# lawmurray/BayesLogit

Measured on NVIDIA B200. Metric: pg_draws_per_sec, higher is better.
Workload: dtype f64

## Files before the change

bayeslogit_b200/api.py:

```python
import ctypes as C

import numpy as np

from . import _lib

NA = float("nan")


def set_seed(seed):
    _lib.lib().bl_set_seed(int(seed) & 0xFFFFFFFFFFFFFFFF)


def set_device(device):
    _lib.check(_lib.lib().bl_set_device(int(device)))


def _recycle(a, num, dtype):
    a = np.asarray(a, dtype=dtype).ravel()
    if a.size != num:
        a = np.resize(a, num)
    return np.ascontiguousarray(a)


def _ptr(a):
# ... 100 lines not shown
    z = np.ascontiguousarray(z, dtype=np.float64)
    shape = np.ascontiguousarray(shape, dtype=dt)
    num = z.size
    x = np.zeros(num)
    t = _lib.Tape()
    keep = []
    for k in "ueng":
        a = tape.get(k)
        if a is None:
            setattr(t, "t" + k, None)
            setattr(t, "l" + k, 0)
        else:
            a = np.ascontiguousarray(a, dtype=np.float64)
            assert a.ndim == 2 and a.shape[0] == num
            keep.append(a)
            setattr(t, "t" + k, a.ctypes.data)
            setattr(t, "l" + k, a.shape[1])
    tr = np.zeros((num, _lib.TRACE_W), dtype=np.int32) if trace else None
    args = [_ptr(x), _ptr(shape), _ptr(z), num]
    it = None
    if method == "gamma":
        args.append(int(trunc))
    if method == "sp":
        it = np.zeros(num, dtype=np.int32)
        args.append(_ptr(it))
    st = getattr(_lib.lib(), fn)(*args, C.byref(t), _ptr(tr) if trace else None)
    _lib.check(st)
    out = [x]
    if trace:
        out.append(tr)
    if it is not None:
        out.append(it)
    return tuple(out) if len(out) > 1 else x


def pg_moments(b, z):
    b = np.ascontiguousarray(b, dtype=np.float64)
    z = np.ascontiguousarray(z, dtype=np.float64)
    m1, m2 = np.zeros(b.size), np.zeros(b.size)
    _lib.check(_lib.lib().bl_probe_pg_moments(_ptr(m1), _ptr(m2), _ptr(b), _ptr(z), b.size))
    return m1, m2


def v_eval(y):
    y = np.ascontiguousarray(y, dtype=np.float64)
    v = np.zeros(y.size)
    _lib.check(_lib.lib().bl_probe_v_eval(_ptr(v), _ptr(y), y.size))
    return v


SPECFUN = {"p_norm": 0, "log_p_norm": 1, "p_gamma_rate": 2, "p_igauss": 3, "lgamma": 4, "tgamma": 5,
           "dev_right_mass": 6, "dev_coef": 7, "upper_gamma_cf": 8, "p_igauss_direct": 9, "sp_log_cos_rt": 10,
           "sp_v_table": 11, "sp_pl": 12, "sp_pl_estimate": 13,
           "alt_pr": 14, "alt_pr_estimate": 15}


def specfun(which, a, b=None, c=None):
    a = np.ascontiguousarray(a, dtype=np.float64)
    b = a if b is None else np.ascontiguousarray(np.broadcast_to(b, a.shape), dtype=np.float64)
    c = a if c is None else np.ascontiguousarray(np.broadcast_to(c, a.shape), dtype=np.float64)
    out = np.zeros(a.size)
    _lib.check(_lib.lib().bl_probe_specfun(_ptr(out), SPECFUN[which], _ptr(a), _ptr(b), _ptr(c), a.size))
    return out


def philox4x32_10(ctr, key):
    ctr = np.ascontiguousarray(ctr, dtype=np.uint32)
    key = np.ascontiguousarray(key, dtype=np.uint32)
    out = np.zeros(4, dtype=np.uint32)
    _lib.check(_lib.lib().bl_probe_philox(_ptr(out), _ptr(ctr), _ptr(key)))
    return out
```

bayeslogit_b200/csrc/pg_alt.cuh:

```cuda
#pragma once

namespace bl {

template <class Src>
__device__ __forceinline__ double alt_rtinvchi2(Src &s, double h, double trunc)
{
    double h2 = h * h;
    double R = trunc / h2;
    double E1 = s.expon();
    double E2 = s.expon();
    while ((E1 * E1) > (2 * E2 / R)) {
        E1 = s.expon();
        E2 = s.expon();
    }
    double X = 1 + E1 * R;
    X = R / (X * X);
    return h2 * X;
}

__device__ __forceinline__ double alt_pigauss(double x, double z, double lambda)
{
    double sq = sqrt(lambda / x);
    double b = sq * (x * z - 1);
    double a = sq * (x * z + 1) * -1.0;
    return p_norm(b) + ool::exp_(2 * lambda * z) * p_norm(a);
}

enum AltField {
    kAltH = 0,
    kAltTrunc,
    kAltPr,
    kAltCoef,
    kAltLgh,
    kAltLd0, kAltLd1,
    kAltLtB, kAltLtC0, kAltLtLM,
    kAltPrBand,
    kAltSetupDoubles
};
constexpr int kAltStateDoubles = 2 * kAltSetupDoubles;

struct AltState {
    double f[kAltStateDoubles];
    __device__ __forceinline__ double get(int k) const { return f[k]; }
};

struct AltStateRef {
    const double *o;
    size_t stride;
    __device__ __forceinline__ double get(int k) const { return o[(size_t)k * stride]; }
};

__device__ __forceinline__ void alt_plan(double h, int &nfull, int &nrem, double &hrem)
{
    double n = floor((h - 1.0) / 4.0);
    double remain = h - 4.0 * n;
    nfull = (int)n;
    if (remain > 4.0) {
        nrem = 2;
        hrem = 0.5 * remain;
    } else {
        nrem = 1;
        hrem = remain;
    }
}

static __device__ __noinline__ double alt_pr_fp64(double h, double z, double trunc)
{
    const double kLog2 = 0.693147180559945309417232;
    double wl, wr;
    if (z != 0)
        wl = ool::exp_(h * (kLog2 - z)) * alt_pigauss(trunc, z / h, h * h);
    else
        wl = ool::exp_(h * kLog2) * (1.0 - p_gamma_rate(1 / trunc, 0.5, 0.5 * h * h));
    double lambda_z = kPi * kPi * 0.125 + 0.5 * z * z;
    wr = ool::exp_(h * ool::log_((0.5 * kPi) / lambda_z)) * (1.0 - p_gamma_rate(trunc, h, lambda_z));
    return wr / (wr + wl);
}

constexpr double kAltPrBandWidth = 2e-5;

__device__ __forceinline__ float alt_pr_estimate(double h, double z, double trunc)
{
    const float hf = (float)h, zf = (float)z, tf = (float)trunc;
    if (!(zf < 12.0f)) return -1.0f;
    const float s = hf * rsqrtf(tf);
    const float tz = tf * zf / hf;
    const float b = s * (tz - 1.0f), na = s * (tz + 1.0f);
    const float phib = 0.5f * erfcf(-b * 0.70710678f);
    const float wl = exp2f(hf) * (__expf(-hf * zf) * phib
                                  + 0.5f * erfcxf(na * 0.70710678f) * __expf(hf * zf - 0.5f * na * na));
    const float lam = 1.2337005501361697f + 0.5f * zf * zf;
    const float x = tf * lam;
    const float lpre = hf * __logf(x) - x;
    float Q;
    if (x < hf + 1.0f) {
        float term = 1.0f, sum = 1.0f, ap = hf;
        for (int k = 0; k < 60; ++k) {
            ap += 1.0f;
            term *= x / ap;
            sum += term;
            if (term < 1e-8f * sum) break;
        }
        Q = 1.0f - sum * __expf(lpre - lgammaf(hf + 1.0f));
    } else {
        float cf = upper_gamma_cf_f32(hf, x);
        if (!(cf > 0.0f)) return -1.0f;
        Q = cf * __expf(lpre - lgammaf(hf));
    }
    if (!(Q > 0.0f)) return -1.0f;
    const float wr = __expf(hf * __logf(1.5707963267948966f / lam)) * Q;
    const float pr = wr / (wr + wl);
    return pr >= 0.0f && pr <= 1.0f ? pr : -1.0f;
}

template <bool kEstimatePr>
static __device__ __noinline__ void alt_setup(double h, double z, double *out)
{
    const double kLog2 = 0.693147180559945309417232;
    int idx = (int)floor((h - 1.0) * 100.0);
    double trunc = PG_TRUNC_SCHEDULE[idx];
    double rate_z = 0.125 * kPi * kPi + 0.5 * z * z;
    float est = kEstimatePr ? alt_pr_estimate(h, z, trunc) : -1.0f;
    out[kAltH] = h;
    out[kAltTrunc] = trunc;
    out[kAltPr] = est >= 0.0f ? (double)est : alt_pr_fp64(h, z, trunc);
    out[kAltPrBand] = est >= 0.0f ? kAltPrBandWidth : 0.0;
    out[kAltCoef] = ool::exp_(h * kLog2 - 0.5 * 1.8378770664093454835606594728112 );
    out[kAltLgh] = ool::lgamma_(h);
    out[kAltLd0] = ool::log_(h);
    out[kAltLd1] = ool::log_(2.0 + h);
    double b = rate_z * trunc;
    double d1 = b - h;
    double d3 = h - 1.0;
    double c0 = 0.5 * (d1 + sqrt(d1 * d1 + 4.0 * b)) / b;
    out[kAltLtB] = b;
    out[kAltLtC0] = c0;
    out[kAltLtLM] = d3 * ool::log_(d3 / (1.0 - c0)) - d3;
}

template <class St>
__device__ __forceinline__ bool alt_pick_right(double u, const St &st, int o, double z)
{
    const double pr = st.get(o + kAltPr), band = st.get(o + kAltPrBand);
    if (u < pr - band) return true;
    if (u > pr + band || band == 0.0) return false;
    return u < alt_pr_fp64(st.get(o + kAltH), z, st.get(o + kAltTrunc));
}

struct AltLane {
    double X, alpha, sum;
    int trial;
    int phase;
    int nfull;
    int nrem;
    __device__ __forceinline__ void start(int nf, int nr)
    {
        X = 0.0; alpha = 0.0; sum = 0.0; trial = 0; phase = 0; nfull = nf; nrem = nr;
    }
};

__device__ __forceinline__ double alt_coef(double n, double lx3, double ldn, double x, double h,
                                           double coef_h, double &g)
{
    double d_n = 2.0 * n + h;
    if (n != 0)
        g *= (n + h - 1) / n;
    else
        g = 1.0;
    double coef = coef_h * g;
    double log_kernel = -0.5 * (lx3 + d_n * d_n / x) + ldn;
    return coef * ool::exp_(log_kernel);
}

template <class Src, class St>
__device__ __forceinline__ bool alt_pick(Src &src, AltLane &L, double z, const St &st)
{
    const int o = L.nfull > 0 ? 0 : kAltSetupDoubles;
    if (L.trial >= 10000) {
        L.sum += -1.0;
        L.trial = 0;
        if (L.nfull > 0)
            L.nfull--;
        else
            L.nrem--;
        return L.nfull == 0 && L.nrem == 0;
    }
    L.trial++;
    if (alt_pick_right(src.unif(), st, o, z)) {
        L.phase = 1;
    } else {
// ... 80 lines not shown
    const double trunc = st.get(o + kAltTrunc);
    bool chunk_done = false;
    double chunk_val = 0.0;
    if (L.phase == 1) {
        double rate_z = 0.125 * kPi * kPi + 0.5 * z * z;
        if (h == 1.0) {
            L.X = src.expon() / rate_z + trunc;
            L.phase = 4;
        } else {
            double b = st.get(o + kAltLtB), c0 = st.get(o + kAltLtC0);
            double x = b + src.expon() / c0;
            double u = src.unif();
            double l_rho = (h - 1.0) * ool::log_(x) - x * (1.0 - c0);
            if (ool::log_(u) <= l_rho - st.get(o + kAltLtLM)) {
                L.X = trunc * (x / b);
                L.phase = 4;
            }
        }
    } else if (L.phase == 2) {
        if (src.unif() > L.alpha) {
            L.X = alt_rtinvchi2(src, h, trunc);
            L.alpha = ool::exp_(-0.5 * z * z * L.X);
        } else {
            L.phase = 4;
        }
    } else if (L.phase == 3) {
        double X = igauss(src, h / z, h * h);
        if (!(X > trunc)) {
            L.X = X;
            L.phase = 4;
        }
    }
    if (L.phase == 4) {
        const double X = L.X;
        const bool accept = alt_series_test(X, src.unif(), h, trunc, st, o);
        L.phase = 0;
        if (accept) {
            chunk_done = true;
            chunk_val = 0.25 * X;
        }
    }
    if (chunk_done) {
        L.sum += chunk_val;
        L.trial = 0;
        if (L.nfull > 0)
            L.nfull--;
        else
            L.nrem--;
        if (L.nfull == 0 && L.nrem == 0) return true;
    }
    return false;
}

template <class Src>
__device__ double alt_draw(Src &s, double h, double z)
{
    if (h < 1) return 0;
    if (h != h) return h;
    int nfull, nrem;
    double hrem;
    alt_plan(h, nfull, nrem, hrem);
    double zh = fabs(z) * 0.5;
    AltState st;
    if (nfull > 0) alt_setup<false>(4.0, zh, st.f);
    alt_setup<false>(hrem, zh, st.f + kAltSetupDoubles);
    AltLane L;
    L.start(nfull, nrem);
    while (!alt_trip(s, L, zh, st)) {}
    return L.sum;
}

}
```

bayeslogit_b200/csrc/pg_hybrid.cu:

```cuda
#include <algorithm>
#include <cstdlib>
#include <vector>

#include "engine.h"
#include "pg_devroye_fast.cuh"
#include "pg_stream.cuh"

namespace bl {

namespace {

constexpr int kBinThreads = 256;
constexpr int kMetaCounts = 0;
constexpr int kMetaOffsets = 8;
constexpr int kMetaCursor = 16;

__global__ void __launch_bounds__(kBinThreads)
k_hyb_count(const double *__restrict__ h, int n, int *__restrict__ meta)
{
    __shared__ int cnt[8];
    if (threadIdx.x < 8) cnt[threadIdx.x] = 0;
    __syncthreads();
    int local[6] = {0, 0, 0, 0, 0, 0};
    for (int i = blockIdx.x * blockDim.x + threadIdx.x; i < n; i += gridDim.x * blockDim.x)
// ... 125 lines not shown
struct RgSlots {
    double f[F][kRgThreads];
    double d[D][kRgThreads];
    uint4 buf[kRgThreads];
    uint32_t blk[kRgThreads];
    int pos[kRgThreads];
    int i[I][kRgThreads];
    int obs[kRgThreads];
    int phase[kRgThreads];
    int perm[kRgThreads];
    int wcnt[kRgThreads / 32][3];
};

struct SpRegroup {
    static constexpr int F = kSpStateDoubles, D = 3, I = 1, kClasses = 2, kRegime = kRegSP;
    using Slots = RgSlots<F, D, I>;
    __device__ static void begin(Slots &S, int t, double shape, double zraw, PhiloxSource &src)
    {
        S.d[0][t] = shape;
        S.d[1][t] = 0.5 * fabs(zraw);
        S.d[2][t] = 2.0;
        S.i[0][t] = 1;
        SpStateRef st{&S.f[0][t], (size_t)kRgThreads};
        S.phase[t] = sp_pick_left(src.unif(), st, shape) ? 1 : 2;
    }
    __device__ static bool advance(Slots &S, int sl, PhiloxSource &src, double &omega)
    {
        SpLane L;
        L.X = S.d[2][sl];
        L.iter = S.i[0][sl];
        L.phase = S.phase[sl];
        const double n = S.d[0][sl];
        SpStateRef st{&S.f[0][sl], (size_t)kRgThreads};
        bool done = sp_trip_staged(src, L, n, S.d[1][sl], st);
        if (!done && L.phase == 0) {
            if (L.iter >= 200) {
                done = true;
            } else {
                L.iter++;
                L.phase = sp_pick_left(src.unif(), st, n) ? 1 : 2;
            }
        }
        if (done) {
            omega = n * 0.25 * L.X;
        } else {
            S.d[2][sl] = L.X;
            S.i[0][sl] = L.iter;
            S.phase[sl] = L.phase;
        }
        return done;
    }
};

struct AltRegroup {
    static constexpr int F = kAltStateDoubles, D = 4, I = 3, kClasses = 3, kRegime = kRegAlt;
    using Slots = RgSlots<F, D, I>;
    __device__ static void load(const Slots &S, int sl, AltLane &L)
    {
        L.X = S.d[1][sl]; L.alpha = S.d[2][sl]; L.sum = S.d[3][sl];
        L.trial = S.i[0][sl]; L.nfull = S.i[1][sl]; L.nrem = S.i[2][sl];
        L.phase = S.phase[sl];
    }
    __device__ static void store(Slots &S, int sl, const AltLane &L)
    {
        S.d[1][sl] = L.X; S.d[2][sl] = L.alpha; S.d[3][sl] = L.sum;
        S.i[0][sl] = L.trial; S.i[1][sl] = L.nfull; S.i[2][sl] = L.nrem;
        S.phase[sl] = L.phase;
    }
    __device__ static void begin(Slots &S, int t, double shape, double zraw, PhiloxSource &src)
    {
        int nfull, nrem;
        double hrem;
        alt_plan(shape, nfull, nrem, hrem);
        AltLane L;
        L.start(nfull, nrem);
        const double zh = 0.5 * fabs(zraw);
        S.d[0][t] = zh;
        AltStateRef st{&S.f[0][t], (size_t)kRgThreads};
        alt_pick(src, L, zh, st);
        store(S, t, L);
    }
    __device__ static bool advance(Slots &S, int sl, PhiloxSource &src, double &omega)
    {
        AltLane L;
        load(S, sl, L);
        const double zh = S.d[0][sl];
        AltStateRef st{&S.f[0][sl], (size_t)kRgThreads};
        bool done = alt_trip<false>(src, L, zh, st);
        while (!done && L.phase == 0) done = alt_pick(src, L, zh, st);
        if (done)
            omega = L.sum;
        else
            store(S, sl, L);
        return done;
    }
};

template <class R, bool kChains = false>
__global__ void __launch_bounds__(kRgThreads)
k_loop_regroup(double *__restrict__ x, const double *__restrict__ h, const double *__restrict__ z,
               const int *__restrict__ idx, const int *__restrict__ meta, const double *__restrict__ state,
               int c0, int cap, StreamId id)
{
    using Slots = typename R::Slots;
    extern __shared__ __align__(16) unsigned char rg_raw[];
    Slots &S = *reinterpret_cast<Slots *>(rg_raw);
    const int count = min(meta[kMetaCounts + R::kRegime] - c0, cap);
    if (count <= 0) return;
    const int *list = idx + meta[kMetaOffsets + R::kRegime] + c0;
    const unsigned full = 0xffffffffu;
    const int t = threadIdx.x, lane = t & 31, warp = t >> 5;
    const unsigned lt_mask = (1u << lane) - 1u;
    constexpr int kWarps = kRgThreads / 32;
    const int gwarp = blockIdx.x * kWarps + warp;
    const int stride = gridDim.x * kWarps * kLaneChunk;
    int cur = gwarp * kLaneChunk, cend = cur + kLaneChunk;

    S.phase[t] = -1;
    __syncthreads();
    for (;;) {
        const bool empty = S.phase[t] < 0;
        const unsigned want = __ballot_sync(full, empty);
        if (want && cur < count) {
            int rank = __popc(want & lt_mask);
            int cand = cur + rank;
            if (cand >= cend) cand += stride - kLaneChunk;
            if (empty && cand < count) {
                const int obs = list[cand];
#pragma unroll
                for (int k = 0; k < R::F; ++k) S.f[k][t] = __ldg(state + (size_t)k * cap + cand);
                S.obs[t] = obs;
                PhiloxSource src;
                if (kChains) open_batch_stream(src, id, obs);
                else src.open(id.seed, id.obs0 + (uint64_t)obs, id.call_id);
                R::begin(S, t, h[obs], z[obs], src);
                S.buf[t] = src.buf;
                S.blk[t] = src.blk;
                S.pos[t] = src.pos;
            }
            cur += __popc(want);
            if (cur >= cend) {
// ... 15 lines not shown
            tot1 += a;
            tot2 += b;
            tot3 += c;
        }
        if (tot1 + tot2 + tot3 == 0) {
            if (!__syncthreads_or(cur < count)) break;
            continue;
        }
        if (ph == 1) S.perm[b1 + __popc(m1 & lt_mask)] = t;
        else if (ph == 3) S.perm[tot1 + b3 + __popc(m3 & lt_mask)] = t;
        else if (ph == 2) S.perm[kRgThreads - 1 - (b2 + __popc(m2 & lt_mask))] = t;
        __syncthreads();
        if (t < tot1 + tot3 || t >= kRgThreads - tot2) {
            const int sl = S.perm[t];
            PhiloxSource src;
            if (kChains) open_batch_stream(src, id, S.obs[sl]);
            else src.open(id.seed, id.obs0 + (uint64_t)S.obs[sl], id.call_id);
            src.buf = S.buf[sl];
            src.blk = S.blk[sl];
            src.pos = S.pos[sl];
            double omega;
            if (R::advance(S, sl, src, omega)) {
                x[S.obs[sl]] = omega;
                S.phase[sl] = -1;
            } else {
                S.buf[sl] = src.buf;
                S.blk[sl] = src.blk;
                S.pos[sl] = src.pos;
            }
        }
        __syncthreads();
    }
}

template <class R, bool kChains>
int regroup_grid()
{
    using Slots = typename R::Slots;
    cudaFuncSetAttribute(k_loop_regroup<R, kChains>, cudaFuncAttributeMaxDynamicSharedMemorySize, (int)sizeof(Slots));
    int per_sm = 0;
    if (cudaOccupancyMaxActiveBlocksPerMultiprocessor(&per_sm, k_loop_regroup<R, kChains>, kRgThreads, sizeof(Slots)) != cudaSuccess || per_sm < 1)
        per_sm = 1;
    int sms = 148, dev = 0;
    if (cudaGetDevice(&dev) == cudaSuccess) cudaDeviceGetAttribute(&sms, cudaDevAttrMultiProcessorCount, dev);
    return sms * per_sm;
}

__global__ void __launch_bounds__(128)
k_alt_setup(const double *__restrict__ h, const double *__restrict__ z, const int *__restrict__ idx,
            const int *__restrict__ meta, double *__restrict__ state, int c0, int cap)
{
    const int count = min(meta[kMetaCounts + kRegAlt] - c0, cap);
    const int *list = idx + meta[kMetaOffsets + kRegAlt] + c0;
    for (int j = blockIdx.x * blockDim.x + threadIdx.x; j < count; j += gridDim.x * blockDim.x) {
        int i = list[j];
        int nfull, nrem;
        double hrem, zh = 0.5 * fabs(z[i]);
        alt_plan(h[i], nfull, nrem, hrem);
        double f[kAltSetupDoubles];
        alt_setup<true>(hrem, zh, f);
#pragma unroll
        for (int k = 0; k < kAltSetupDoubles; ++k) state[(size_t)(kAltSetupDoubles + k) * cap + j] = f[k];
        if (nfull > 0) {
            alt_setup<true>(4.0, zh, f);
#pragma unroll
            for (int k = 0; k < kAltSetupDoubles; ++k) state[(size_t)k * cap + j] = f[k];
        }
    }
}

constexpr int kStateChunk = 1 << 23;
constexpr int kStateDoubles = kSpStateDoubles > kAltStateDoubles ? kSpStateDoubles : kAltStateDoubles;

template <class K>
int resident_grid(K kernel, int threads, int need)
{
    int per_sm = 0;
    if (cudaOccupancyMaxActiveBlocksPerMultiprocessor(&per_sm, kernel, threads, 0) != cudaSuccess || per_sm < 1)
        per_sm = 1;
    int sms = 148;
    int dev = 0;
    if (cudaGetDevice(&dev) == cudaSuccess) cudaDeviceGetAttribute(&sms, cudaDevAttrMultiProcessorCount, dev);
    int cap = sms * per_sm;
    return need < cap ? (need > 0 ? need : 1) : cap;
}

template <int R, bool kChains>
void launch_regime(double *x, const double *h, const double *z, const int *idx, const int *meta,
                   StreamId id, int n, cudaStream_t st)
{
    static const int cap = resident_grid(k_hyb_regime<R, kChains>, 128, 1 << 30);
    int need = (n + 127) / 128;
    k_hyb_regime<R, kChains><<<need < cap ? need : cap, 128, 0, st>>>(x, h, z, idx, meta, id);
    count_launch();
}

}

enum HybStage { kStBin = 0, kStSpSetup, kStSpLoop, kStAltSetup, kStAltLoop, kStGamma, kStNormal, kStDevroye, kStCount };
static bool g_hyb_timing = false;
static std::vector<cudaEvent_t> g_hyb_pool;
struct HybSpan { int stage; int a, b; };
static std::vector<HybSpan> g_hyb_spans;
static int g_hyb_used = 0;

void hybrid_timing_enable(bool on) { g_hyb_timing = on; }

static int hyb_mark(cudaStream_t st)
{
    if ((int)g_hyb_pool.size() <= g_hyb_used) {
        cudaEvent_t e;
        cudaEventCreate(&e);
        g_hyb_pool.push_back(e);
    }
    cudaEventRecord(g_hyb_pool[g_hyb_used], st);
    return g_hyb_used++;
}

struct HybTimer {
    bool on;
    cudaStream_t st;
    int stage, a;
    HybTimer(bool on_, cudaStream_t st_, int stage_) : on(on_), st(st_), stage(stage_), a(on_ ? hyb_mark(st_) : 0) {}
    ~HybTimer() { if (on) g_hyb_spans.push_back(HybSpan{stage, a, hyb_mark(st)}); }
};

int hybrid_timing_last(double *ms8, int *launches8)
{
    if (g_hyb_spans.empty()) return 1;
    for (int k = 0; k < kStCount; ++k) { ms8[k] = 0.0; if (launches8) launches8[k] = 0; }
    if (cudaEventSynchronize(g_hyb_pool[g_hyb_used - 1]) != cudaSuccess) return 1;
    for (const HybSpan &sp : g_hyb_spans) {
        float ms = 0.f;
        cudaEventElapsedTime(&ms, g_hyb_pool[sp.a], g_hyb_pool[sp.b]);
        ms8[sp.stage] += ms;
        if (launches8 && ms > 0.02f) launches8[sp.stage]++;
    }
    return 0;
}

static size_t hybrid_state_offset(int64_t num) { return ((32 + (size_t)num) * sizeof(int) + 15) / 16 * 16; }

size_t hybrid_workspace_bytes(int64_t num)
{
    size_t cap = (size_t)(num < kStateChunk ? num : kStateChunk);
    return hybrid_state_offset(num) + cap * kStateDoubles * sizeof(double);
}

struct SideStream {
    cudaStream_t s = nullptr;
    cudaEvent_t fork = nullptr, join = nullptr;
    cudaStream_t get()
    {
        if (!s) {
            int lo = 0, hi = 0;
            cudaDeviceGetStreamPriorityRange(&lo, &hi);
            cudaStreamCreateWithPriority(&s, cudaStreamNonBlocking, lo);
            cudaEventCreateWithFlags(&fork, cudaEventDisableTiming);
            cudaEventCreateWithFlags(&join, cudaEventDisableTiming);
        }
        return s;
    }
};
static SideStream g_side;

template <bool kChains>
static cudaError_t launch_hybrid_binned_k(double *x, const double *h, const double *z, int num, StreamId id,
                                          void *work, cudaStream_t st)
{
    if (num <= 0) return cudaSuccess;
    int *meta = (int *)work;
    int *idx = meta + 32;
    cudaError_t e = cudaMemsetAsync(meta, 0, 32 * sizeof(int), st);
    if (e != cudaSuccess) return e;
    int tiles = (num + kBinThreads - 1) / kBinThreads;
    int grid = tiles < 148 * 8 ? tiles : 148 * 8;
    int stiles = (num + kBinThreads * kBinPer - 1) / (kBinThreads * kBinPer);
    int sgrid = stiles < 148 * 8 ? stiles : 148 * 8;
    const bool tm = g_hyb_timing;
    if (tm) { g_hyb_spans.clear(); g_hyb_used = 0; }
    {
        HybTimer t(tm, st, kStBin);
        k_hyb_count<<<grid, kBinThreads, 0, st>>>(h, num, meta);
        k_hyb_offsets<<<1, 1, 0, st>>>(meta);
        k_hyb_scatter<<<sgrid, kBinThreads, 0, st>>>(h, num, meta, idx, x);
        count_launch(3);
    }
    static const bool use_side = getenv("BL_HYBRID_NO_SIDE_STREAM") == nullptr;
    cudaStream_t side = use_side ? g_side.get() : st;
    if (use_side) {
        cudaEventRecord(g_side.fork, st);
        cudaStreamWaitEvent(side, g_side.fork, 0);
    }
    {
        HybTimer t(tm, side, kStGamma);
        launch_regime<kRegGamma, kChains>(x, h, z, idx, meta, id, num, side);
    }
    {
        HybTimer t(tm, side, kStNormal);
        launch_regime<kRegNormal, kChains>(x, h, z, idx, meta, id, num, side);
    }
    {
        HybTimer t(tm, side, kStDevroye);
        launch_regime<kRegDevroye, kChains>(x, h, z, idx, meta, id, num, side);
    }
    double *state = (double *)((char *)work + hybrid_state_offset(num));
    const int cap = num < kStateChunk ? num : kStateChunk;
    static const int g_sp_setup = resident_grid(k_sp_setup, 128, 1 << 30);
    static const int g_alt_setup = resident_grid(k_alt_setup, 128, 1 << 30);
    static const int g_sp_regroup = regroup_grid<SpRegroup, kChains>();
    static const int g_alt_regroup = regroup_grid<AltRegroup, kChains>();
    const int rneed = (cap + kLaneChunk * (kRgThreads / 32) - 1) / (kLaneChunk * (kRgThreads / 32));
    const int sneed = (cap + 127) / 128;
    for (int c0 = 0; c0 < num; c0 += cap) {
        {
            HybTimer t(tm, st, kStSpSetup);
            k_sp_setup<<<std::min(sneed, g_sp_setup), 128, 0, st>>>(h, z, idx, meta, state, c0, cap);
        }
        {
            HybTimer t(tm, st, kStSpLoop);
            k_loop_regroup<SpRegroup, kChains><<<std::min(rneed, g_sp_regroup), kRgThreads, sizeof(SpRegroup::Slots), st>>>(x, h, z, idx, meta, state, c0, cap, id);
        }
        count_launch(2);
    }
    for (int c0 = 0; c0 < num; c0 += cap) {
        {
            HybTimer t(tm, st, kStAltSetup);
            k_alt_setup<<<std::min(sneed, g_alt_setup), 128, 0, st>>>(h, z, idx, meta, state, c0, cap);
        }
        {
            HybTimer t(tm, st, kStAltLoop);
            k_loop_regroup<AltRegroup, kChains><<<std::min(rneed, g_alt_regroup), kRgThreads, sizeof(AltRegroup::Slots), st>>>(x, h, z, idx, meta, state, c0, cap, id);
        }
        count_launch(2);
    }
    if (use_side) {
        cudaEventRecord(g_side.join, side);
        cudaStreamWaitEvent(st, g_side.join, 0);
    }
    return cudaGetLastError();
}

cudaError_t launch_hybrid_binned(double *x, const double *h, const double *z, int num, StreamId id,
                                 void *work, cudaStream_t st)
{
    return id.chain_len ? launch_hybrid_binned_k<true>(x, h, z, num, id, work, st)
                        : launch_hybrid_binned_k<false>(x, h, z, num, id, work, st);
}

}
```

bayeslogit_b200/csrc/pg_kernels.cu:

```cuda
#include "engine.h"
#include "pg_devroye_fast.cuh"
#include "pg_stream.cuh"

namespace bl {

namespace {

constexpr int kThreads = 128;

inline int grid_for(int64_t num, int threads, int ctas_per_sm)
{
    int64_t need = (num + threads - 1) / threads;
    int64_t cap = 148LL * ctas_per_sm;
    return (int)(need < cap ? (need > 0 ? need : 1) : cap);
}

template <int M, class Src>
__device__ __forceinline__ double draw_one(Src &s, const void *shape, const double *z, int64_t i,
                                           int trunc, int *iter, int &aux)
{
    aux = 0;
    if (M == kDevroye || M == kDevroyeLoop) {
        int n = ((const int *)shape)[i];
        return n != 0 ? devroye_sum_fast(s, n, z[i]) : 0.0;
// ... 45 lines not shown
    for (int64_t i = (int64_t)blockIdx.x * blockDim.x + threadIdx.x; i < num; i += stride) {
        TapeSource s;
        s.open(tp.tu, tp.lu, tp.te, tp.le, tp.tn, tp.ln, tp.tg, tp.lg, (size_t)i);
        int aux;
        double v = draw_one<M>(s, shape, z, i, trunc, iter, aux);
        x[i] = s.exhausted() ? nan("") : v;
        if (trace) {
            int *t = trace + i * BL_TRACE_W;
            s.counts(t);
            t[4] = s.exhausted() ? 1 : 0;
            t[5] = aux;
        }
    }
}

__global__ void k_probe_moments(double *m1, double *m2, const double *b, const double *z, int64_t num)
{
    int64_t i = (int64_t)blockIdx.x * blockDim.x + threadIdx.x;
    if (i < num) {
        m1[i] = pg_m1(b[i], z[i]);
        m2[i] = pg_m2(b[i], z[i]);
    }
}

__global__ void k_probe_v_eval(double *v, const double *y, int64_t num)
{
    int64_t i = (int64_t)blockIdx.x * blockDim.x + threadIdx.x;
    if (i < num) v[i] = v_eval(y[i]);
}

__global__ void k_probe_specfun(double *out, int which, const double *a, const double *b,
                                const double *c, int64_t num)
{
    int64_t i = (int64_t)blockIdx.x * blockDim.x + threadIdx.x;
    if (i >= num) return;
    double r = 0.0;
    switch (which) {
    case 0: r = p_norm(a[i]); break;
    case 1: r = log_p_norm(a[i]); break;
    case 2: r = p_gamma_rate(a[i], b[i], c[i]); break;
    case 3: r = p_igauss(a[i], b[i], c[i]); break;
    case 4: r = lgamma(a[i]); break;
    case 5: r = tgamma(a[i]); break;
    case 6: r = dev_right_mass(a[i]); break;
    case 7: r = dev_coef((int)b[i], a[i]); break;
    case 8: r = upper_gamma_cf(b[i], a[i]); break;
    case 9: r = p_igauss_direct(a[i], b[i], c[i]); break;
    case 10: { double v, g; sp_vg(a[i], v, g); r = g; break; }
    case 11: { double v, g; r = sp_vg_table(a[i], v, g) ? v : nan(""); break; }
    case 12: { SpState st; sp_setup<false>(a[i], b[i], st); r = st.f[kSpPl]; break; }
    case 13: { SpState st; sp_setup<true>(a[i], b[i], st); r = st.f[kSpPlBand] > 0.0 ? st.f[kSpPl] : nan(""); break; }
    case 14: { double f[kAltSetupDoubles]; alt_setup<false>(a[i], 0.5 * fabs(b[i]), f); r = f[kAltPr]; break; }
    case 15: { double f[kAltSetupDoubles]; alt_setup<true>(a[i], 0.5 * fabs(b[i]), f); r = f[kAltPrBand] > 0.0 ? f[kAltPr] : nan(""); break; }
    }
    out[i] = r;
}

__global__ void k_probe_philox(uint32_t *out4, const uint32_t *ctr4, const uint32_t *key2)
{
    uint4 r = Philox4x32::block(make_uint4(ctr4[0], ctr4[1], ctr4[2], ctr4[3]),
                                make_uint2(key2[0], key2[1]));
    out4[0] = r.x; out4[1] = r.y; out4[2] = r.z; out4[3] = r.w;
}

template <int M, bool kChains = false>
cudaError_t launch_philox_m(double *x, const void *shape, const double *z, int64_t num, int trunc,
                            int *iter, StreamId id, cudaStream_t st)
{
    if (num <= 0) return cudaSuccess;
    k_rpg_philox<M, kChains><<<grid_for(num, kThreads, 16), kThreads, 0, st>>>(x, shape, z, num, trunc, iter, id);
    count_launch();
    return cudaGetLastError();
}

template <int M>
cudaError_t launch_tape_m(double *x, const void *shape, const double *z, int64_t num, int trunc,
                          int *iter, DevTape tp, int *trace, cudaStream_t st)
{
    if (num <= 0) return cudaSuccess;
    k_rpg_tape<M><<<grid_for(num, kThreads, 16), kThreads, 0, st>>>(x, shape, z, num, trunc, iter, tp, trace);
    count_launch();
    return cudaGetLastError();
}

}

cudaError_t launch_rpg(Method m, double *x, const void *shape, const double *z, int64_t num,
                       int trunc, int *iter, StreamId id, cudaStream_t st)
{
    switch (m) {
    case kDevroye: return launch_devroye_refill(x, (const int *)shape, z, num, id, st);
    case kDevroyeLoop: return launch_philox_m<kDevroyeLoop>(x, shape, z, num, trunc, iter, id, st);
    case kGamma: return launch_philox_m<kGamma>(x, shape, z, num, trunc, iter, id, st);
    case kAlt: return launch_philox_m<kAlt>(x, shape, z, num, trunc, iter, id, st);
    case kSP: return launch_philox_m<kSP>(x, shape, z, num, trunc, iter, id, st);
    case kHybrid:
        return id.chain_len ? launch_philox_m<kHybrid, true>(x, shape, z, num, trunc, iter, id, st)
                            : launch_philox_m<kHybrid>(x, shape, z, num, trunc, iter, id, st);
    case kDevroyePlain: return launch_philox_m<kDevroyePlain>(x, shape, z, num, trunc, iter, id, st);
    }
    return cudaErrorInvalidValue;
}

cudaError_t launch_rpg_tape(Method m, double *x, const void *shape, const double *z, int64_t num,
                            int trunc, int *iter, DevTape tp, int *trace, cudaStream_t st)
{
// ... 48 lines not shown
```

bayeslogit_b200/csrc/pg_samplers.cuh:

```cuda
#pragma once

#include "philox.cuh"
#include "specfun.cuh"

#define PG_TABLE_QUAL static __device__ __constant__
#include "pg_tables.h"

namespace bl {

constexpr double kTrunc = 0.64;

namespace ool {
static __device__ __noinline__ double log_(double x) { return ::log(x); }
static __device__ __noinline__ double exp_(double x) { return ::exp(x); }
static __device__ __noinline__ double tan_(double x) { return ::tan(x); }
static __device__ __noinline__ double tanh_(double x) { return ::tanh(x); }
static __device__ __noinline__ double cos_(double x) { return ::cos(x); }
static __device__ __noinline__ double cosh_(double x) { return ::cosh(x); }
static __device__ __noinline__ double atan_(double x) { return ::atan(x); }
static __device__ __noinline__ double lgamma_(double x) { return ::lgamma(x); }
static __device__ __noinline__ double tgamma_(double x) { return ::tgamma(x); }
}


// ... 140 lines not shown
{
    z = fabs(z);
    if (z > 1e-12) return b * tanh(z) / z;
    return b * (1 - (1.0 / 3) * pow(z, 2) + (2.0 / 15) * pow(z, 4) - (17.0 / 315) * pow(z, 6));
}

__device__ __forceinline__ double jj_m2(double b, double z)
{
    z = fabs(z);
    if (z > 1e-12) {
        double tz = tanh(z) / z;
        return (b + 1) * b * (tz * tz) + b * ((tanh(z) - z) / (z * z * z));
    }
    double p = 1 - (1.0 / 3) * pow(z, 2) + (2.0 / 15) * pow(z, 4) - (17.0 / 315) * pow(z, 6);
    return (b + 1) * b * (p * p) + b * ((-1.0 / 3) + (2.0 / 15) * pow(z, 2) - (17.0 / 315) * pow(z, 4));
}

__device__ __forceinline__ double pg_m1(double b, double z) { return jj_m1(b, 0.5 * z) * 0.25; }
__device__ __forceinline__ double pg_m2(double b, double z) { return jj_m2(b, 0.5 * z) * 0.0625; }


template <class Src>
__device__ __forceinline__ double igauss(Src &s, double mu, double lambda)
{
    double nu = s.norm();
    double y = nu * nu;
    double x = mu + 0.5 * mu * mu * y / lambda
             - 0.5 * mu / lambda * sqrt(4.0 * mu * lambda * y + (mu * y) * (mu * y));
    if (s.unif() > mu / (mu + x)) x = mu * mu / x;
    return x;
}

template <class Src>
__device__ __noinline__ double ltgamma(Src &s, double shape, double rate, double trunc)
{
    double a = shape;
    double b = rate * trunc;
    if (trunc <= 0.0 || shape < 1.0) return 0.0;
    if (shape == 1.0) return s.expon() / rate + trunc;
    double d1 = b - a;
    double d3 = a - 1.0;
    double c0 = 0.5 * (d1 + sqrt(d1 * d1 + 4.0 * b)) / b;
    double l_M = d3 * ool::log_(d3 / (1.0 - c0)) - d3;
    double x;
    for (;;) {
        x = b + s.expon() / c0;
        double u = s.unif();
        double l_rho = d3 * ool::log_(x) - x * (1.0 - c0);
        if (ool::log_(u) <= l_rho - l_M) break;
    }
    return trunc * (x / b);
}

template <class Src>
__device__ __forceinline__ double tnorm_left(Src &s, double left)
{
    if (left < 0.0) {
        for (;;) {
            double z = s.norm();
            if (z > left) return z;
        }
    }
    double astar = 0.5 * (left + sqrt(left * left + 4.0));
    for (;;) {
        double z = s.expon() / astar + left;
        double rho = ool::exp_(-0.5 * (z - astar) * (z - astar));
        if (s.unif() < rho) return z;
    }
}

template <class Src>
__device__ __forceinline__ double rtinvchi2(Src &s, double scale, double trunc)
{
    double R = trunc / scale;
    double z = tnorm_left(s, 1.0 / sqrt(R));
    return scale / (z * z);
}

}

#include "pg_alt.cuh"
#include "pg_sp.cuh"

namespace bl {


enum Regime { kRegZero = 0, kRegGamma = 1, kRegDevroye = 2, kRegAlt = 3, kRegSP = 4, kRegNormal = 5 };

__device__ __forceinline__ int regime_of(double b)
{
    if (b > 170) return kRegNormal;
    if (b > 13) return kRegSP;
    if (b == 1 || b == 2) return kRegDevroye;
    if (b > 1) return kRegAlt;
    if (b > 0) return kRegGamma;
    return kRegZero;
}

template <class Src>
__device__ double devroye_sum_fast(Src &s, int n, double z);

template <class Src>
__device__ double hybrid_draw(Src &s, double b, double z, int &aux)
{
    aux = 0;
    switch (regime_of(b)) {
// ... 23 lines not shown
```

bayeslogit_b200/csrc/pg_sp.cuh:

```cuda
#pragma once

#include "pg_sp_tables.h"

namespace bl {

__device__ __forceinline__ double y_of_v(double v, double tol)
{
    double r = sqrt(fabs(v));
    if (v > tol) return ool::tan_(r) / r;
    if (v < -1 * tol) return ool::tanh_(r) / r;
    return 1.0;
}

static __device__ __noinline__ double v_eval_ref(double y)
{
    const double tol = 1e-9;
    const int max_iter = 1000;
    if (y < PG_YGRID[0]) return -1. / (y * y);
    if (y > PG_YGRID[PG_YGRID_LEN - 1]) {
        double v = ool::atan_(0.5 * y * kPi);
        return v * v;
    }
    if (y == 1) return 0.0;
    double id = (ool::log_(y) / ool::log_(2.0) + 4.0) / 0.1;
// ... 291 lines not shown
        if (L.iter >= maxiter) return true;
        L.iter++;
        L.phase = sp_pick_left(src.unif(), s, n) ? 1 : 2;
    }
    if (L.phase == 1) {
        double mu = 1. / s.get(kSpRt2rl);
        if (md < mu) {
            double X = md + 1.0, alpha = 0.0;
            while (src.unif() > alpha) {
                X = rtinvchi2(src, n, md);
                alpha = ool::exp_(-0.5 * n / (mu * mu) * X);
            }
            L.X = X;
            L.phase = 3;
        } else {
            double X = igauss(src, mu, n);
            if (!(X > md)) {
                L.X = X;
                L.phase = 3;
            }
        }
    } else if (L.phase == 2) {
        if (n > 1.0 && md > 0.0) {
            double b = s.get(kSpLtB), c0 = s.get(kSpLtC0);
            double x = b + src.expon() / c0;
            double u = src.unif();
            double l_rho = (n - 1.0) * ool::log_(x) - x * (1.0 - c0);
            if (ool::log_(u) <= l_rho - s.get(kSpLtLM)) {
                L.X = md * (x / b);
                L.phase = 4;
            }
        } else {
            L.X = ltgamma(src, n, n * s.get(kSpRr), md);
            L.phase = 4;
        }
    }
    if (L.phase >= 3) {
        double X = L.X, F;
        if (L.phase == 3) {
            double phi_ev = n * (s.get(kSpIl) - s.get(kSpRl) * X) + 0.5 * n * ((1. - 1. / X) - (1. - 1. / md));
            F = ool::exp_(s.get(kSpCl) - 1.5 * ool::log_(X) + phi_ev);
        } else {
            double phi_ev = n * (s.get(kSpIr) - s.get(kSpRr) * X) + n * (ool::log_(X) - s.get(kSpLmd));
            F = ool::exp_(s.get(kSpCr) + phi_ev) / X;
        }
        double spa = sp_density(X, n, z, s);
        if (F * src.unif() < spa) return true;
        L.phase = 0;
        if (L.iter >= maxiter) return true;
    }
    return false;
}

static __device__ __noinline__ bool sp_ltgamma_accept_exact(double u, double x, double n, double c0, double l_M)
{
    return ool::log_(u) <= (n - 1.0) * ool::log_(x) - x * (1.0 - c0) - l_M;
}

template <class St>
static __device__ __noinline__ bool sp_accept_exact(double X, bool left, double n, double z, double u,
                                                    const St &s)
{
    double F;
    if (left) {
        double phi_ev = n * (s.get(kSpIl) - s.get(kSpRl) * X) + 0.5 * n * ((1. - 1. / X) - (1. - 1. / s.get(kSpMd)));
        F = ool::exp_(s.get(kSpCl) - 1.5 * ool::log_(X) + phi_ev);
    } else {
        double phi_ev = n * (s.get(kSpIr) - s.get(kSpRr) * X) + n * (ool::log_(X) - s.get(kSpLmd));
        F = ool::exp_(s.get(kSpCr) + phi_ev) / X;
    }
    return F * u < sp_density(X, n, z, s);
}

template <class St>
__device__ __forceinline__ bool sp_trip_staged(PhiloxSource &src, SpLane &L, double n, double z, const St &s)
{
    const int maxiter = 200;
    const double md = s.get(kSpMd);
    const double mu = s.get(kSpMu);
    if (!(n > 1.0 && md > 0.0 && md >= mu)) {
        PhiloxSource tsrc = src;
        SpLane tl = L;
        bool r = sp_trip(tsrc, tl, n, z, s);
        src = tsrc;
        L = tl;
        return r;
    }
    if (L.phase == 0) {
        if (L.iter >= maxiter) return true;
        L.iter++;
        L.phase = sp_pick_left(src.unif(), s, n) ? 1 : 2;
    }
    const bool left = L.phase == 1;
    PhiloxSource::LazyN ln = {0u, 0u, 0u};
    PhiloxSource::LazyE le = {0u, 0};
    double a1;
    if (left) {
        ln = src.norm_lazy();
        uint64_t m = ((uint64_t)ln.w0 << 21) | (uint64_t)(ln.w1 >> 11);
        a1 = ((double)m + 0.5) * 0x1p-53;
    } else {
        le = src.expon_lazy();
        a1 = word_to_unif(le.w);
    }
    const double L1 = ool::log_(a1);
    const double u = src.unif();
    double X;
    bool ok;
    float lx;
    if (left) {
        double nu = sqrt(-2.0 * L1) * cospi(2.0 * word_to_unif(ln.w2));
        double y = nu * nu;
        double x = mu + 0.5 * mu * mu * y / n - 0.5 * mu / n * sqrt(4.0 * mu * n * y + (mu * y) * (mu * y));
        if (u > mu / (mu + x)) x = mu * mu / x;
        X = x;
        ok = !(X > md);
        lx = __logf((float)X);
    } else {
        double E = (double)le.k * (32.0 * 0.693147180559945309417232) - L1;
        double c0 = s.get(kSpLtC0), b = s.get(kSpLtB);
        double xg = b + E / c0;
        lx = __logf((float)xg);
        float lu = __logf((float)u);
        double d = (n - 1.0) * (double)lx - xg * (1.0 - c0) - s.get(kSpLtLM) - (double)lu;
        double band = 1e-6 * ((n - 1.0) * (1.0 + fabs((double)lx)) + 2.0 + fabs((double)lu));
        if (d > band) ok = true;
        else if (d < -band) ok = false;
        else ok = sp_ltgamma_accept_exact(u, xg, n, c0, s.get(kSpLtLM));
        X = md * (xg / b);
    }
    if (!ok) return false;
    L.X = X;
    const double u2 = src.unif();
    double logX, logF, kx;
    if (left) {
        logX = (double)lx;
        logF = s.get(kSpCl) - 1.5 * logX + n * (s.get(kSpIl) - s.get(kSpRl) * X)
             + 0.5 * n * ((1. - 1. / X) - s.get(kSpC1md));
        kx = 1.5;
    } else {
        double dl = (double)lx - s.get(kSpLLtB);
        logX = s.get(kSpLmd) + dl;
        logF = s.get(kSpCr) + n * (s.get(kSpIr) - s.get(kSpRr) * X) + n * dl - logX;
        kx = n + 1.0;
    }
    double v, g;
    sp_vg(X, v, g);
    double t = 0.5 * v + 0.5 * (z * z);
    double phi = s.get(kSpLcz) - g - t * X;
    double K2 = fabs(v) >= 1e-6 ? X * X + (1 - X) / v : X * X;
    float lK2 = __logf((float)K2);
    double log_spa = s.get(kSpLcn) - 0.5 * (double)lK2 + n * phi;
    double a = log_spa - logF;
    bool accept;
    if (fabs(logF) < 700.0 && fabs(log_spa) < 700.0) {
        double band = 1e-6 * (kx * (1.0 + fabs((double)lx)) + 0.5 * (1.0 + fabs((double)lK2)));
        if (a >= band) {
            accept = true;
        } else {
            double thr = (double)__expf((float)a);
            double rb = band + 5e-7 * (1.0 + fabs(a));
            if (u2 < thr * (1.0 - rb)) accept = true;
            else if (u2 > thr * (1.0 + rb)) accept = false;
            else accept = sp_accept_exact(X, left, n, z, u2, s);
        }
    } else {
        accept = sp_accept_exact(X, left, n, z, u2, s);
    }
    if (accept) return true;
    L.phase = 0;
    return L.iter >= maxiter;
}

template <class Src>
__device__ int sp_draw(Src &src, double &d, double n, double z)
{
    SpState s;
    sp_setup(n, z, s);
    SpLane L;
    L.start();
    double zh = 0.5 * fabs(z);
// ... 7 lines not shown
```

Baseline: 5.067 billion.

## Overlap alt regime on its own stream and stage its rejection tests

Moves the alt-regime setup and loop kernels onto a separate side stream so they run concurrently with the saddle-point regime instead of after it. The per-sample alt state shrinks by hoisting the z-independent fields for shape 4 into one global table computed once. Alt trips now use lazy exponentials with a float-first banded accept/reject test that falls back to exact fp64 only near the boundary, reusing the staged lt-gamma test shared with the SP sampler. This adds extra workspace, so alt and SP state no longer alias, plus the risk of a race on the global table, which is written by a single thread while other blocks read it.

```diff
diff --git a/bayeslogit_b200/api.py b/bayeslogit_b200/api.py
--- a/bayeslogit_b200/api.py
+++ b/bayeslogit_b200/api.py
@@ -176,7 +176,7 @@
 SPECFUN = {"p_norm": 0, "log_p_norm": 1, "p_gamma_rate": 2, "p_igauss": 3, "lgamma": 4, "tgamma": 5,
            "dev_right_mass": 6, "dev_coef": 7, "upper_gamma_cf": 8, "p_igauss_direct": 9, "sp_log_cos_rt": 10,
            "sp_v_table": 11, "sp_pl": 12, "sp_pl_estimate": 13,
-           "alt_pr": 14, "alt_pr_estimate": 15}
+           "alt_pr": 14, "alt_pr_estimate": 15, "alt_setup_field": 16, "alt_zfree_field": 17}
 
 
 def specfun(which, a, b=None, c=None):
diff --git a/bayeslogit_b200/csrc/pg_alt.cuh b/bayeslogit_b200/csrc/pg_alt.cuh
--- a/bayeslogit_b200/csrc/pg_alt.cuh
+++ b/bayeslogit_b200/csrc/pg_alt.cuh
@@ -29,25 +29,33 @@
 enum AltField {
     kAltH = 0,
     kAltTrunc,
-    kAltPr,
     kAltCoef,
     kAltLgh,
     kAltLd0, kAltLd1,
+    kAltZFree,
+    kAltPr = kAltZFree,
+    kAltPrBand,
     kAltLtB, kAltLtC0, kAltLtLM,
-    kAltPrBand,
     kAltSetupDoubles
 };
-constexpr int kAltStateDoubles = 2 * kAltSetupDoubles;
 
 struct AltState {
-    double f[kAltStateDoubles];
+    double f[2 * kAltSetupDoubles];
     __device__ __forceinline__ double get(int k) const { return f[k]; }
 };
+
+constexpr int kAltStateDoubles = 2 * kAltSetupDoubles - kAltZFree;
 
 struct AltStateRef {
     const double *o;
     size_t stride;
-    __device__ __forceinline__ double get(int k) const { return o[(size_t)k * stride]; }
+    const double *c4;
+    __device__ __forceinline__ double get(int k) const
+    {
+        if (k >= kAltSetupDoubles) return o[(size_t)(k - kAltSetupDoubles) * stride];
+        if (k < kAltZFree) return __ldg(c4 + k);
+        return o[(size_t)(k + kAltSetupDoubles - kAltZFree) * stride];
+    }
 };
 
 __device__ __forceinline__ void alt_plan(double h, int &nfull, int &nrem, double &hrem)
@@ -113,22 +121,25 @@
     return pr >= 0.0f && pr <= 1.0f ? pr : -1.0f;
 }
 
-template <bool kEstimatePr>
-static __device__ __noinline__ void alt_setup(double h, double z, double *out)
+static __device__ __noinline__ void alt_setup_zfree(double h, double *out)
 {
     const double kLog2 = 0.693147180559945309417232;
     int idx = (int)floor((h - 1.0) * 100.0);
-    double trunc = PG_TRUNC_SCHEDULE[idx];
-    double rate_z = 0.125 * kPi * kPi + 0.5 * z * z;
-    float est = kEstimatePr ? alt_pr_estimate(h, z, trunc) : -1.0f;
     out[kAltH] = h;
-    out[kAltTrunc] = trunc;
-    out[kAltPr] = est >= 0.0f ? (double)est : alt_pr_fp64(h, z, trunc);
-    out[kAltPrBand] = est >= 0.0f ? kAltPrBandWidth : 0.0;
+    out[kAltTrunc] = PG_TRUNC_SCHEDULE[idx];
     out[kAltCoef] = ool::exp_(h * kLog2 - 0.5 * 1.8378770664093454835606594728112 );
     out[kAltLgh] = ool::lgamma_(h);
     out[kAltLd0] = ool::log_(h);
     out[kAltLd1] = ool::log_(2.0 + h);
+}
+
+template <bool kEstimatePr>
+static __device__ __noinline__ void alt_setup_z(double h, double z, double trunc, double *out)
+{
+    double rate_z = 0.125 * kPi * kPi + 0.5 * z * z;
+    float est = kEstimatePr ? alt_pr_estimate(h, z, trunc) : -1.0f;
+    out[kAltPr] = est >= 0.0f ? (double)est : alt_pr_fp64(h, z, trunc);
+    out[kAltPrBand] = est >= 0.0f ? kAltPrBandWidth : 0.0;
     double b = rate_z * trunc;
     double d1 = b - h;
     double d3 = h - 1.0;
@@ -136,6 +147,13 @@
     out[kAltLtB] = b;
     out[kAltLtC0] = c0;
     out[kAltLtLM] = d3 * ool::log_(d3 / (1.0 - c0)) - d3;
+}
+
+template <bool kEstimatePr>
+__device__ __forceinline__ void alt_setup(double h, double z, double *out)
+{
+    alt_setup_zfree(h, out);
+    alt_setup_z<kEstimatePr>(h, z, out[kAltTrunc], out);
 }
 
 template <class St>
@@ -322,6 +340,115 @@
     return false;
 }
 
+static __device__ __noinline__ bool alt_rtinvchi2_reject_exact(uint32_t w1, int k1, uint32_t w2, int k2, double R)
+{
+    const double E1 = PhiloxSource::exact(PhiloxSource::LazyE{w1, k1});
+    const double E2 = PhiloxSource::exact(PhiloxSource::LazyE{w2, k2});
+    return (E1 * E1) > (2 * E2 / R);
+}
+
+__device__ __forceinline__ PhiloxSource::LazyE alt_rtinvchi2_e1(PhiloxSource &src, double R)
+{
+    const double r2 = 2.0 / R;
+    for (;;) {
+        const PhiloxSource::LazyE e1 = src.expon_lazy();
+        const PhiloxSource::LazyE e2 = src.expon_lazy();
+        bool reject;
+        if ((e1.k | e2.k) == 0) {
+            const double f1 = (double)PhiloxSource::approx(e1), f2 = (double)PhiloxSource::approx(e2);
+            const double t1 = 1e-6 * (1.0 + f1), t2 = 1e-6 * (1.0 + f2);
+            const double d = f1 * f1 - r2 * f2;
+            const double band = (2.0 * f1 + t1) * t1 + r2 * t2;
+            if (d > band) reject = true;
+            else if (d < -band) reject = false;
+            else reject = alt_rtinvchi2_reject_exact(e1.w, e1.k, e2.w, e2.k, R);
+        } else {
+            reject = alt_rtinvchi2_reject_exact(e1.w, e1.k, e2.w, e2.k, R);
+        }
+        if (!reject) return e1;
+    }
+}
+
+template <class St>
+__device__ __forceinline__ bool alt_trip_staged(PhiloxSource &src, AltLane &L, double z, const St &st)
+{
+    const int o = L.nfull > 0 ? 0 : kAltSetupDoubles;
+    const double h = st.get(o + kAltH);
+    const double trunc = st.get(o + kAltTrunc);
+    bool need = true;
+    double a1 = 0.5;
+    int k = 0;
+    uint32_t wn2 = 0u;
+    if (L.phase == 1) {
+        const PhiloxSource::LazyE e = src.expon_lazy();
+        a1 = word_to_unif(e.w);
+        k = e.k;
+    } else if (L.phase == 2) {
+        need = src.unif() > L.alpha;
+        if (need) {
+            const PhiloxSource::LazyE e = alt_rtinvchi2_e1(src, trunc / (h * h));
+            a1 = word_to_unif(e.w);
+            k = e.k;
+        } else {
+            L.phase = 4;
+        }
+    } else {
+        const PhiloxSource::LazyN n = src.norm_lazy();
+        const uint64_t m = ((uint64_t)n.w0 << 21) | (uint64_t)(n.w1 >> 11);
+        a1 = ((double)m + 0.5) * 0x1p-53;
+        wn2 = n.w2;
+    }
+    double L1 = 0.0;
+    if (need) L1 = ool::log_(a1);
+    const double E = (double)k * (32.0 * 0.693147180559945309417232) - L1;
+    if (L.phase == 1) {
+        if (h == 1.0) {
+            double rate_z = 0.125 * kPi * kPi + 0.5 * z * z;
+            L.X = E / rate_z + trunc;
+            L.phase = 4;
+        } else {
+            const double b = st.get(o + kAltLtB), c0 = st.get(o + kAltLtC0);
+            const double x = b + E / c0;
+            const double u = src.unif();
+            float lx;
+            if (ltgamma_accept_staged(u, x, h, c0, st.get(o + kAltLtLM), lx)) {
+                L.X = trunc * (x / b);
+                L.phase = 4;
+            }
+        }
+    } else if (L.phase == 2) {
+        double h2 = h * h;
+        double R = trunc / h2;
+        double X = 1 + E * R;
+        X = R / (X * X);
+        L.X = h2 * X;
+        L.alpha = ool::exp_(-0.5 * z * z * L.X);
+    } else if (L.phase == 3) {
+        const double mu = h / z, lambda = h * h;
+        double nu = sqrt(-2.0 * L1) * cospi(2.0 * word_to_unif(wn2));
+        double y = nu * nu;
+        double x = mu + 0.5 * mu * mu * y / lambda
+                 - 0.5 * mu / lambda * sqrt(4.0 * mu * lambda * y + (mu * y) * (mu * y));
+        if (src.unif() > mu / (mu + x)) x = mu * mu / x;
+        if (!(x > trunc)) {
+            L.X = x;
+            L.phase = 4;
+        }
+    }
+    if (L.phase != 4) return false;
+    const double X = L.X;
+    const bool accept = alt_series_test(X, src.unif(), h, trunc, st, o);
+    L.phase = 0;
+    if (!accept) return false;
+    L.sum += 0.25 * X;
+    L.trial = 0;
+    if (L.nfull > 0)
+        L.nfull--;
+    else
+        L.nrem--;
+    return L.nfull == 0 && L.nrem == 0;
+}
+
 template <class Src>
 __device__ double alt_draw(Src &s, double h, double z)
 {
diff --git a/bayeslogit_b200/csrc/pg_hybrid.cu b/bayeslogit_b200/csrc/pg_hybrid.cu
--- a/bayeslogit_b200/csrc/pg_hybrid.cu
+++ b/bayeslogit_b200/csrc/pg_hybrid.cu
@@ -201,6 +201,8 @@
     }
 };
 
+__device__ double g_alt_shape4[kAltZFree];
+
 struct AltRegroup {
     static constexpr int F = kAltStateDoubles, D = 4, I = 3, kClasses = 3, kRegime = kRegAlt;
     using Slots = RgSlots<F, D, I>;
@@ -225,7 +227,7 @@
         L.start(nfull, nrem);
         const double zh = 0.5 * fabs(zraw);
         S.d[0][t] = zh;
-        AltStateRef st{&S.f[0][t], (size_t)kRgThreads};
+        AltStateRef st{&S.f[0][t], (size_t)kRgThreads, g_alt_shape4};
         alt_pick(src, L, zh, st);
         store(S, t, L);
     }
@@ -234,8 +236,8 @@
         AltLane L;
         load(S, sl, L);
         const double zh = S.d[0][sl];
-        AltStateRef st{&S.f[0][sl], (size_t)kRgThreads};
-        bool done = alt_trip<false>(src, L, zh, st);
+        AltStateRef st{&S.f[0][sl], (size_t)kRgThreads, g_alt_shape4};
+        bool done = alt_trip_staged(src, L, zh, st);
         while (!done && L.phase == 0) done = alt_pick(src, L, zh, st);
         if (done)
             omega = L.sum;
@@ -357,6 +359,8 @@
 {
     const int count = min(meta[kMetaCounts + kRegAlt] - c0, cap);
     const int *list = idx + meta[kMetaOffsets + kRegAlt] + c0;
+    if (c0 == 0 && blockIdx.x == 0 && threadIdx.x == 0) alt_setup_zfree(4.0, g_alt_shape4);
+    const double trunc4 = PG_TRUNC_SCHEDULE[300];
     for (int j = blockIdx.x * blockDim.x + threadIdx.x; j < count; j += gridDim.x * blockDim.x) {
         int i = list[j];
         int nfull, nrem;
@@ -365,17 +369,16 @@
         double f[kAltSetupDoubles];
         alt_setup<true>(hrem, zh, f);
 #pragma unroll
-        for (int k = 0; k < kAltSetupDoubles; ++k) state[(size_t)(kAltSetupDoubles + k) * cap + j] = f[k];
+        for (int k = 0; k < kAltSetupDoubles; ++k) state[(size_t)k * cap + j] = f[k];
         if (nfull > 0) {
-            alt_setup<true>(4.0, zh, f);
-#pragma unroll
-            for (int k = 0; k < kAltSetupDoubles; ++k) state[(size_t)k * cap + j] = f[k];
+            alt_setup_z<true>(4.0, zh, trunc4, f);
+#pragma unroll
+            for (int k = kAltZFree; k < kAltSetupDoubles; ++k) state[(size_t)(kAltSetupDoubles + k - kAltZFree) * cap + j] = f[k];
         }
     }
 }
 
 constexpr int kStateChunk = 1 << 23;
-constexpr int kStateDoubles = kSpStateDoubles > kAltStateDoubles ? kSpStateDoubles : kAltStateDoubles;
 
 template <class K>
 int resident_grid(K kernel, int threads, int need)
@@ -434,8 +437,8 @@
 {
     if (g_hyb_spans.empty()) return 1;
     for (int k = 0; k < kStCount; ++k) { ms8[k] = 0.0; if (launches8) launches8[k] = 0; }
-    if (cudaEventSynchronize(g_hyb_pool[g_hyb_used - 1]) != cudaSuccess) return 1;
     for (const HybSpan &sp : g_hyb_spans) {
+        if (cudaEventSynchronize(g_hyb_pool[sp.b]) != cudaSuccess) return 1;
         float ms = 0.f;
         cudaEventElapsedTime(&ms, g_hyb_pool[sp.a], g_hyb_pool[sp.b]);
         ms8[sp.stage] += ms;
@@ -449,7 +452,7 @@
 size_t hybrid_workspace_bytes(int64_t num)
 {
     size_t cap = (size_t)(num < kStateChunk ? num : kStateChunk);
-    return hybrid_state_offset(num) + cap * kStateDoubles * sizeof(double);
+    return hybrid_state_offset(num) + cap * (kSpStateDoubles + kAltStateDoubles) * sizeof(double);
 }
 
 struct SideStream {
@@ -467,7 +470,7 @@
         return s;
     }
 };
-static SideStream g_side;
+static SideStream g_side, g_alt_side;
 
 template <bool kChains>
 static cudaError_t launch_hybrid_binned_k(double *x, const double *h, const double *z, int num, StreamId id,
@@ -493,9 +496,11 @@
     }
     static const bool use_side = getenv("BL_HYBRID_NO_SIDE_STREAM") == nullptr;
     cudaStream_t side = use_side ? g_side.get() : st;
+    cudaStream_t alt = use_side ? g_alt_side.get() : st;
     if (use_side) {
         cudaEventRecord(g_side.fork, st);
         cudaStreamWaitEvent(side, g_side.fork, 0);
+        cudaStreamWaitEvent(alt, g_side.fork, 0);
     }
     {
         HybTimer t(tm, side, kStGamma);
@@ -509,8 +514,9 @@
         HybTimer t(tm, side, kStDevroye);
         launch_regime<kRegDevroye, kChains>(x, h, z, idx, meta, id, num, side);
     }
+    const int cap = num < kStateChunk ? num : kStateChunk;
     double *state = (double *)((char *)work + hybrid_state_offset(num));
-    const int cap = num < kStateChunk ? num : kStateChunk;
+    double *alt_state = state + (size_t)kSpStateDoubles * cap;
     static const int g_sp_setup = resident_grid(k_sp_setup, 128, 1 << 30);
     static const int g_alt_setup = resident_grid(k_alt_setup, 128, 1 << 30);
     static const int g_sp_regroup = regroup_grid<SpRegroup, kChains>();
@@ -519,6 +525,17 @@
     const int sneed = (cap + 127) / 128;
     for (int c0 = 0; c0 < num; c0 += cap) {
         {
+            HybTimer t(tm, alt, kStAltSetup);
+            k_alt_setup<<<std::min(sneed, g_alt_setup), 128, 0, alt>>>(h, z, idx, meta, alt_state, c0, cap);
+        }
+        {
+            HybTimer t(tm, alt, kStAltLoop);
+            k_loop_regroup<AltRegroup, kChains><<<std::min(rneed, g_alt_regroup), kRgThreads, sizeof(AltRegroup::Slots), alt>>>(x, h, z, idx, meta, alt_state, c0, cap, id);
+        }
+        count_launch(2);
+    }
+    for (int c0 = 0; c0 < num; c0 += cap) {
+        {
             HybTimer t(tm, st, kStSpSetup);
             k_sp_setup<<<std::min(sneed, g_sp_setup), 128, 0, st>>>(h, z, idx, meta, state, c0, cap);
         }
@@ -528,20 +545,11 @@
         }
         count_launch(2);
     }
-    for (int c0 = 0; c0 < num; c0 += cap) {
-        {
-            HybTimer t(tm, st, kStAltSetup);
-            k_alt_setup<<<std::min(sneed, g_alt_setup), 128, 0, st>>>(h, z, idx, meta, state, c0, cap);
-        }
-        {
-            HybTimer t(tm, st, kStAltLoop);
-            k_loop_regroup<AltRegroup, kChains><<<std::min(rneed, g_alt_regroup), kRgThreads, sizeof(AltRegroup::Slots), st>>>(x, h, z, idx, meta, state, c0, cap, id);
-        }
-        count_launch(2);
-    }
     if (use_side) {
         cudaEventRecord(g_side.join, side);
         cudaStreamWaitEvent(st, g_side.join, 0);
+        cudaEventRecord(g_alt_side.join, alt);
+        cudaStreamWaitEvent(st, g_alt_side.join, 0);
     }
     return cudaGetLastError();
 }
diff --git a/bayeslogit_b200/csrc/pg_kernels.cu b/bayeslogit_b200/csrc/pg_kernels.cu
--- a/bayeslogit_b200/csrc/pg_kernels.cu
+++ b/bayeslogit_b200/csrc/pg_kernels.cu
@@ -121,6 +121,14 @@
     case 13: { SpState st; sp_setup<true>(a[i], b[i], st); r = st.f[kSpPlBand] > 0.0 ? st.f[kSpPl] : nan(""); break; }
     case 14: { double f[kAltSetupDoubles]; alt_setup<false>(a[i], 0.5 * fabs(b[i]), f); r = f[kAltPr]; break; }
     case 15: { double f[kAltSetupDoubles]; alt_setup<true>(a[i], 0.5 * fabs(b[i]), f); r = f[kAltPrBand] > 0.0 ? f[kAltPr] : nan(""); break; }
+    case 16: {
+        double f[kAltSetupDoubles]; int k = (int)c[i];
+        alt_setup<false>(a[i], 0.5 * fabs(b[i]), f); r = k >= 0 && k < kAltSetupDoubles ? f[k] : nan(""); break;
+    }
+    case 17: {
+        double f[kAltZFree]; int k = (int)c[i];
+        alt_setup_zfree(a[i], f); r = k >= 0 && k < kAltZFree ? f[k] : nan(""); break;
+    }
     }
     out[i] = r;
 }
diff --git a/bayeslogit_b200/csrc/pg_samplers.cuh b/bayeslogit_b200/csrc/pg_samplers.cuh
--- a/bayeslogit_b200/csrc/pg_samplers.cuh
+++ b/bayeslogit_b200/csrc/pg_samplers.cuh
@@ -216,6 +216,22 @@
     return trunc * (x / b);
 }
 
+static __device__ __noinline__ bool ltgamma_accept_exact(double u, double x, double n, double c0, double l_M)
+{
+    return ool::log_(u) <= (n - 1.0) * ool::log_(x) - x * (1.0 - c0) - l_M;
+}
+
+__device__ __forceinline__ bool ltgamma_accept_staged(double u, double x, double n, double c0, double l_M, float &lx)
+{
+    lx = __logf((float)x);
+    const float lu = __logf((float)u);
+    const double d = (n - 1.0) * (double)lx - x * (1.0 - c0) - l_M - (double)lu;
+    const double band = 1e-6 * ((n - 1.0) * (1.0 + fabs((double)lx)) + 2.0 + fabs((double)lu));
+    if (d > band) return true;
+    if (d < -band) return false;
+    return ltgamma_accept_exact(u, x, n, c0, l_M);
+}
+
 template <class Src>
 __device__ __forceinline__ double tnorm_left(Src &s, double left)
 {
diff --git a/bayeslogit_b200/csrc/pg_sp.cuh b/bayeslogit_b200/csrc/pg_sp.cuh
--- a/bayeslogit_b200/csrc/pg_sp.cuh
+++ b/bayeslogit_b200/csrc/pg_sp.cuh
@@ -367,11 +367,6 @@
     return false;
 }
 
-static __device__ __noinline__ bool sp_ltgamma_accept_exact(double u, double x, double n, double c0, double l_M)
-{
-    return ool::log_(u) <= (n - 1.0) * ool::log_(x) - x * (1.0 - c0) - l_M;
-}
-
 template <class St>
 static __device__ __noinline__ bool sp_accept_exact(double X, bool left, double n, double z, double u,
                                                     const St &s)
@@ -435,13 +430,7 @@
         double E = (double)le.k * (32.0 * 0.693147180559945309417232) - L1;
         double c0 = s.get(kSpLtC0), b = s.get(kSpLtB);
         double xg = b + E / c0;
-        lx = __logf((float)xg);
-        float lu = __logf((float)u);
-        double d = (n - 1.0) * (double)lx - xg * (1.0 - c0) - s.get(kSpLtLM) - (double)lu;
-        double band = 1e-6 * ((n - 1.0) * (1.0 + fabs((double)lx)) + 2.0 + fabs((double)lu));
-        if (d > band) ok = true;
-        else if (d < -band) ok = false;
-        else ok = sp_ltgamma_accept_exact(u, xg, n, c0, s.get(kSpLtLM));
+        ok = ltgamma_accept_staged(u, xg, n, c0, s.get(kSpLtLM), lx);
         X = md * (xg / b);
     }
     if (!ok) return false;
```

New measurement: 5.145 billion, median of 6. 1.02x the previous value.
